# ZhiHuangHn/vtkCloudPoint

Measured on AMD Instinct MI355X. Metric: Mpoints/s DBSCAN+label @10M pts, higher is better.
Workload: dtype f64; 1 GPU; C4: 10000000-pt cloud (half uniform background, 200 Gaussian blobs), one monolithic DBImproved.dbscan, metric L1_2D, eps 0.1, minPts 10; mode=single, points_total=10000000, points_per_gpu=10000000, clusters=27380, resident_in_hbm=True

## Files before the change

vtkcloudpoint_amd/csrc/gridbuild.hip:

```cpp
#include <algorithm>
#include <mutex>
#include <unordered_map>
#include <vector>

#include "grid_common.hpp"
#include "wave.hpp"

using namespace vcpg;

namespace {

constexpr int PT = 1024;
constexpr int PCH_MIN = 8192;
constexpr int FT = 1024;
constexpr uint32_t MAXB = 8192;
constexpr uint32_t wcap(int) { return 4096u; }
constexpr uint32_t QUEUE_FROM = 32;

typedef float4 Rec;

template <int GD>
__device__ __forceinline__ Rec rec_make(const float* qf, uint32_t idx, uint32_t cell) {
  return GD == 2 ? make_float4(qf[0], qf[1], __uint_as_float(idx), __uint_as_float(cell))
                 : make_float4(qf[0], qf[1], qf[2], __uint_as_float(idx));
}
template <int GD>
__device__ __forceinline__ uint32_t rec_cell(const Rec& r, const GridP& g, uint32_t& idx) {
  if (GD == 2) {
    idx = __float_as_uint(r.z);
    return __float_as_uint(r.w);
  }
  idx = __float_as_uint(r.w);
  const float qf[3] = {r.x, r.y, r.z};
  int cc[3];
  return cell_of32<3>(qf, g, cc);
}

template <int GD>
__device__ __forceinline__ uint32_t coords_cell(const double* q, const GridP& g, float* qf) {
  int cc[3];
#pragma unroll
  for (int a = 0; a < GD; a++) qf[a] = rel32(q[a], g.mn[a], g.scale);
  return cell_of32<GD>(qf, g, cc);
}
template <int GD>
__device__ __forceinline__ uint32_t point_cell(const double* __restrict__ c, int64_t i, int stride, const GridP& g, float* qf) {
  double q[3];
  load_in<GD>(c, i, stride, q);
  return coords_cell<GD>(q, g, qf);
}

struct PartGeom {
  uint32_t csh;
  uint32_t B;
  uint32_t a;
  uint32_t NS;
  uint32_t chunk;
  uint32_t nchunk;
};

inline int env_int(const char* name, int dflt, int lo, int hi) {
  const char* e = getenv(name);
  int v = e ? atoi(e) : dflt;
  return v < lo ? lo : v > hi ? hi : v;
}

inline PartGeom part_geom(int64_t n, uint32_t ncells) {
  static const int csh_max = env_int("VCP_CPB_LOG2", 14, 10, 14);
  static const int target = env_int("VCP_PART_CHUNKS", 256, 64, 8192);
  PartGeom p;
  int csh = csh_max;
  while (csh > 10 && ((uint64_t)ncells >> csh) * 4096ull < (uint64_t)n) csh--;
  p.csh = (uint32_t)csh;
  p.B = (uint32_t)((((uint64_t)ncells + 1) + ((1ull << p.csh) - 1)) >> p.csh);
  p.a = 0;
  while (((p.B + (1u << p.a) - 1u) >> p.a) > MAXB) p.a++;
  p.NS = (p.B + (1u << p.a) - 1u) >> p.a;
  int64_t chunk = (n + target - 1) / target;
  if (chunk < PCH_MIN) chunk = PCH_MIN;
  chunk = (chunk + PT - 1) / PT * PT;
  p.chunk = (uint32_t)chunk;
  p.nchunk = (uint32_t)((n + chunk - 1) / chunk);
  return p;
}

template <int GD, bool GROUPED>
__global__ __launch_bounds__(PT) void k_part_hist(const double* __restrict__ c, int64_t n, int stride, GridP g,
                                                 const int32_t* __restrict__ group, int glo, int ghi, uint32_t csh,
                                                 uint32_t B, uint32_t chunk, uint32_t nchunk,
                                                 uint32_t* __restrict__ counts, uint32_t* __restrict__ qcount,
                                                 uint32_t* __restrict__ ctcount) {
  extern __shared__ uint32_t h[];
  if (blockIdx.x == 0 && threadIdx.x == 0) {
    *qcount = 0u;
    ctcount[0] = 0u;
  }
  for (uint32_t k = threadIdx.x; k < B; k += PT) h[k] = 0;
  __syncthreads();
  const int64_t first = (int64_t)blockIdx.x * chunk;
  const int64_t last = min(first + (int64_t)chunk, n);
#pragma unroll 4
  for (int64_t i = first + threadIdx.x; i < last; i += PT) {
    if (GROUPED) {
      const int gg = group[i];
      if (gg < glo || gg >= ghi) continue;
    }
    float qf[3];
    atomicAdd(&h[point_cell<GD>(c, i, stride, g, qf) >> csh], 1u);
  }
  __syncthreads();
  for (uint32_t k = threadIdx.x; k < B; k += PT) counts[(size_t)k * nchunk + blockIdx.x] = h[k];
}

template <int GD, bool GROUPED>
__global__ __launch_bounds__(PT) void k_part_scatter(const double* __restrict__ c, int64_t n, int stride, GridP g,
                                                    const int32_t* __restrict__ group, int glo, int ghi, uint32_t csh,
                                                    uint32_t B, uint32_t chunk, uint32_t nchunk,
                                                    const uint32_t* __restrict__ base, Rec* __restrict__ rec,
                                                    uint32_t* __restrict__ pos) {
  extern __shared__ uint32_t h[];
  for (uint32_t k = threadIdx.x; k < B; k += PT) h[k] = base[(size_t)k * nchunk + blockIdx.x];
  __syncthreads();
  const int64_t first = (int64_t)blockIdx.x * chunk;
  const int64_t last = min(first + (int64_t)chunk, n);
#pragma unroll 4
  for (int64_t i = first + threadIdx.x; i < last; i += PT) {
    if (GROUPED) {
      const int gg = group[i];
      if (gg < glo || gg >= ghi) {
        if (pos) pos[i] = NONE;
        continue;
      }
    }
    float qf[3];
    const uint32_t cell = point_cell<GD>(c, i, stride, g, qf);
    rec[atomicAdd(&h[cell >> csh], 1u)] = rec_make<GD>(qf, (uint32_t)i, cell);
  }
}

constexpr size_t PAIR_LDS = sizeof(Rec) + 8;
constexpr size_t LDS_CU = 160 * 1024;

template <int GD, bool GROUPED>
__global__ __launch_bounds__(PT) void k_part_scatter_pairs(const double* __restrict__ c, int64_t n, int stride, GridP g,
                                                          const int32_t* __restrict__ group, int glo, int ghi, uint32_t csh,
                                                          uint32_t B, uint32_t chunk, uint32_t nchunk,
                                                          const uint32_t* __restrict__ base, Rec* __restrict__ rec,
                                                          uint32_t* __restrict__ pos) {
  extern __shared__ __attribute__((aligned(16))) unsigned char lds[];
  Rec* stash = reinterpret_cast<Rec*>(lds);
  uint32_t* h = reinterpret_cast<uint32_t*>(stash + B);
  uint32_t* stash_slot = h + B;
  for (uint32_t k = threadIdx.x; k < B; k += PT) {
    h[k] = base[(size_t)k * nchunk + blockIdx.x];
    stash_slot[k] = NONE;
  }
  __syncthreads();
  const int64_t first = (int64_t)blockIdx.x * chunk;
  const int64_t last = min(first + (int64_t)chunk, n);
  const uint32_t trips = first < last ? (uint32_t)((last - first + PT - 1) / PT) : 0u;
  double nq[3] = {0.0, 0.0, 0.0};
  bool ntake = false;
  auto fetch = [&](int64_t i) {
    ntake = i < last;
    if (GROUPED && ntake) {
      const int gg = group[i];
      if (gg < glo || gg >= ghi) {
        if (pos) pos[i] = NONE;
        ntake = false;
      }
    }
    if (ntake) load_in<GD>(c, i, stride, nq);
  };
  fetch(first + threadIdx.x);
  for (uint32_t t = 0; t < trips; t++) {
    const int64_t i = first + (int64_t)t * PT + threadIdx.x;
    const bool take = ntake;
    const double q[3] = {nq[0], nq[1], nq[2]};
    fetch(i + PT);
    Rec r = make_float4(0.0f, 0.0f, 0.0f, 0.0f);
    uint32_t b = 0, slot = 0;
    if (take) {
      float qf[3];
      const uint32_t cell = coords_cell<GD>(q, g, qf);
      r = rec_make<GD>(qf, (uint32_t)i, cell);
      b = cell >> csh;
      slot = atomicAdd(&h[b], 1u);
    }
    __syncthreads();
    bool keep = false;
    if (take) {
      if (slot & 1u) {
        if (stash_slot[b] == slot - 1u) rec[slot - 1u] = stash[b];
        rec[slot] = r;
      } else if (h[b] > slot + 1u) {
        rec[slot] = r;
      } else {
        keep = true;
      }
    }
    __syncthreads();
    if (keep) {
      stash[b] = r;
      stash_slot[b] = slot;
    }
  }
  __syncthreads();
  for (uint32_t k = threadIdx.x; k < B; k += PT) {
    const uint32_t s = stash_slot[k];
    if (s != NONE && h[k] == s + 1u) rec[s] = stash[k];
  }
}

__device__ __forceinline__ uint32_t padded(uint32_t i) { return i + (i >> 5); }

template <int GD, bool GROUPED, int NT = FT>
__device__ __forceinline__ void fine_flush(uint32_t s0, uint32_t m, const float* s32, const uint32_t* sidx,
                                           const uint32_t* __restrict__ ord, const uint8_t* __restrict__ in_classed,
                                           const int32_t* __restrict__ group, float* __restrict__ sorted32,
                                           uint32_t* __restrict__ sord, uint32_t* __restrict__ sidx_out,
                                           int32_t* __restrict__ sgroup, uint8_t* __restrict__ flags,
                                           uint32_t* __restrict__ pos) {
  if (GD == 2) {
    const float2* src = reinterpret_cast<const float2*>(s32);
    float2* dst = reinterpret_cast<float2*>(sorted32) + s0;
    for (uint32_t k = threadIdx.x; k < m; k += NT) dst[k] = src[k];
  } else {
    const float4* src = reinterpret_cast<const float4*>(s32);
    float4* dst = reinterpret_cast<float4*>(sorted32) + s0;
    for (uint32_t k = threadIdx.x; k < m; k += NT) dst[k] = src[k];
  }
  for (uint32_t k = threadIdx.x; k < m; k += NT) {
    const uint32_t i = sidx[k], p = s0 + k;
    sord[p] = ord ? ord[i] : i;
    if (sidx_out) sidx_out[p] = i;
    if (GROUPED) sgroup[p] = group[i];
    if (in_classed) flags[p] = in_classed[i] ? F_CLASSED : 0;
    if (pos) pos[i] = p;
  }
}

template <int GD>
__device__ __forceinline__ void stage_put(float* s32, uint32_t* sidx, uint32_t p, const Rec& r, uint32_t idx) {
  if (GD == 2) reinterpret_cast<float2*>(s32)[p] = make_float2(r.x, r.y);
  else reinterpret_cast<float4*>(s32)[p] = make_float4(r.x, r.y, r.z, 0.0f);
  sidx[p] = idx;
}

__device__ __forceinline__ void bucket_range(const uint32_t* __restrict__ bstart, uint32_t bstride, const uint32_t* __restrict__ total,
                                             uint32_t b, uint32_t B, uint32_t& s, uint32_t& e) {
  s = bstart[(size_t)b * bstride];
  e = (b + 1 < B) ? bstart[(size_t)(b + 1) * bstride] : *total;
}

template <int GD>
__global__ __launch_bounds__(FT) void k_part_split(const Rec* __restrict__ rec, Rec* __restrict__ rec2,
                                                  const uint32_t* __restrict__ base, const uint32_t* __restrict__ total,
                                                  uint32_t nchunk, uint32_t NS, uint32_t a, uint32_t csh, uint32_t B, GridP g,
                                                  uint32_t* __restrict__ bstart) {
  __shared__ uint32_t h[32];
  const uint32_t S = blockIdx.x;
  uint32_t s, e;
  bucket_range(base, nchunk, total, S, NS, s, e);
  const uint32_t subm = (1u << a) - 1u;
  if (threadIdx.x < 32) h[threadIdx.x] = 0u;
  __syncthreads();
  for (uint32_t j = s + threadIdx.x; j < e; j += FT) {
    uint32_t i;
    atomicAdd(&h[(rec_cell<GD>(rec[j], g, i) >> csh) & subm], 1u);
  }
  __syncthreads();
  if (threadIdx.x < 32) {
    const uint32_t v = h[threadIdx.x];
    const uint32_t inc = wave_incl<WaveAdd, 32>(v, (int)threadIdx.x);
    const uint32_t first = s + inc - v;
    h[threadIdx.x] = first;
    const uint32_t bk = (S << a) + threadIdx.x;
    if (threadIdx.x <= subm && bk <= B) bstart[bk] = first;
  }
  __syncthreads();
  for (uint32_t j = s + threadIdx.x; j < e; j += FT) {
    const Rec r = rec[j];
    uint32_t i;
    rec2[atomicAdd(&h[(rec_cell<GD>(r, g, i) >> csh) & subm], 1u)] = r;
  }
}

constexpr int FS = 512;
constexpr uint32_t scap(int gd) { return gd == 2 ? 2048u : 1536u; }
constexpr uint32_t SPOP = 128;

template <int GD, bool GROUPED>
__global__ __launch_bounds__(FS) void k_part_fine_small(const Rec* __restrict__ rec, const uint32_t* __restrict__ bstart,
                                                       uint32_t bstride, const uint32_t* __restrict__ total, uint32_t B,
                                                       uint32_t csh, GridP g, const uint32_t* __restrict__ ord,
                                                       const uint8_t* __restrict__ in_classed, const int32_t* __restrict__ group,
                                                       uint4* __restrict__ ctwords, uint32_t* __restrict__ ctdense,
                                                       uint32_t* __restrict__ ctcount, uint8_t* __restrict__ bstate,
                                                       float* __restrict__ sorted32, uint32_t* __restrict__ sord,
                                                       uint32_t* __restrict__ sidx_out, int32_t* __restrict__ sgroup,
                                                       uint8_t* __restrict__ flags, uint32_t* __restrict__ pos) {
  constexpr uint32_t FPR = GD == 2 ? 2 : 4;
  constexpr uint32_t SCAP = scap(GD);
  constexpr int SRPT = SCAP / FS;
  __shared__ uint32_t ws[512 + 2];
  __shared__ uint32_t wlo[512], whi[512];
  __shared__ uint16_t wpi[512];
  __shared__ uint8_t sci[SCAP];
  __shared__ __attribute__((aligned(16))) uint16_t st32[SPOP][32];
  __shared__ __attribute__((aligned(16))) float s32[SCAP * FPR];
  __shared__ uint32_t sidx[SCAP];
  __shared__ uint32_t wsum[FS / 64];
  __shared__ uint32_t s_np, s_dbase;
  const uint32_t b = blockIdx.x;
  uint32_t s, e;
  bucket_range(bstart, bstride, total, b, B, s, e);
  const uint32_t m = e - s;
  if (b + 1 == B && threadIdx.x == 0) ctcount[1] = *total;
  if (m > SCAP) {
    if (threadIdx.x == 0) bstate[b] = 1;
    return;
  }
  const uint32_t CPB = 1u << csh, NW = CPB >> 5, c0 = b << csh;
  const int lane = threadIdx.x & 63, w = threadIdx.x >> 6;
  for (uint32_t k = threadIdx.x; k < NW + 1; k += FS) ws[k] = 0u;
  __syncthreads();
  Rec r[SRPT];
  uint32_t idx[SRPT], lw[SRPT], ci[SRPT], rnk[SRPT];
#pragma unroll
  for (int k = 0; k < SRPT; k++) {
    const uint32_t j = s + (uint32_t)k * FS + threadIdx.x;
    lw[k] = NONE;
    if (j < e) {
      r[k] = rec[j];
      const uint32_t c = rec_cell<GD>(r[k], g, idx[k]) - c0;
      lw[k] = c >> 5;
      ci[k] = c & 31u;
      rnk[k] = atomicAdd(&ws[lw[k]], 1u);
    }
  }
  __syncthreads();
  {
    const uint32_t v = threadIdx.x < NW ? ws[threadIdx.x] : 0u;
    const uint32_t inc = wave_incl<WaveAdd>(v, lane);
    if (lane == 63) wsum[w] = inc;
    __syncthreads();
    uint32_t pre = inc - v;
    for (int k = 0; k < w; k++) pre += wsum[k];
    if (threadIdx.x < NW) ws[threadIdx.x] = s + pre;
    if (threadIdx.x == 0) ws[NW] = e;
  }
  __syncthreads();
#pragma unroll
  for (int k = 0; k < SRPT; k++)
    if (lw[k] != NONE) sci[ws[lw[k]] - s + rnk[k]] = (uint8_t)ci[k];
  __syncthreads();
  bool popl = false;
  uint32_t lo = 0u, hi = 0u;
  if (threadIdx.x < NW) {
    const uint32_t a = ws[threadIdx.x] - s, k = ws[threadIdx.x + 1] - s - a;
    if (k > 64u) {
      popl = true;
    } else {
      for (uint32_t i = 0; i < k; i++) {
        const uint32_t bit = 1u << sci[a + i];
        if (lo & hi & bit) continue;
        if (lo & bit) hi ^= bit;
        lo ^= bit;
      }
      popl = (lo & hi) != 0u;
    }
  }
  {
    uint32_t tot;
    const uint32_t before = block_rank<FS>(popl, wsum, tot);
    if (threadIdx.x == 0) s_np = tot;
    if (threadIdx.x < NW) wpi[threadIdx.x] = popl ? (uint16_t)before : (uint16_t)0xFFFFu;
  }
  __syncthreads();
  const uint32_t np = s_np;
  if (np > SPOP) {
    if (threadIdx.x == 0) bstate[b] = 1;
    return;
  }
  if (threadIdx.x == 0) {
    bstate[b] = 0;
    s_dbase = np ? atomicAdd(&ctcount[0], np) : 0u;
  }
  for (uint32_t k = threadIdx.x; k < np * 16u; k += FS) reinterpret_cast<uint32_t*>(&st32[0][0])[k] = 0u;
  if (threadIdx.x < NW && !popl) {
    wlo[threadIdx.x] = lo;
    whi[threadIdx.x] = hi;
  }
  __syncthreads();
#pragma unroll
  for (int k = 0; k < SRPT; k++)
    if (lw[k] != NONE && wpi[lw[k]] != 0xFFFFu) {
      uint16_t* c = &st32[wpi[lw[k]]][ci[k]];
      atomicAdd(reinterpret_cast<uint32_t*>(reinterpret_cast<uintptr_t>(c) & ~(uintptr_t)3), ((uintptr_t)c & 2) ? 0x10000u : 1u);
    }
  __syncthreads();
  {
    const uint32_t hw = threadIdx.x >> 5, li = threadIdx.x & 31u;
    for (uint32_t wd = hw; wd < NW; wd += FS / 32) {
      const uint32_t pi = wpi[wd];
      if (pi == 0xFFFFu) continue;
      const uint32_t c = st32[pi][li];
      uint32_t inc = c;
#pragma unroll
      for (int d = 1; d < 32; d <<= 1) {
        const uint32_t t = __shfl_up(inc, d, 32);
        if ((int)li >= d) inc += t;
      }
      const uint32_t first = ws[wd] + inc - c;
      st32[pi][li] = (uint16_t)(first - s);
      ctdense[(size_t)(s_dbase + pi) * 32u + li] = first;
      const uint32_t cs = min(c, 3u);
      const unsigned long long blo = __ballot(cs & 1u), bhi = __ballot(cs >> 1);
      const int sh = (threadIdx.x & 32) ? 32 : 0;
      if (li == 0) {
        wlo[wd] = (uint32_t)(blo >> sh);
        whi[wd] = (uint32_t)(bhi >> sh);
      }
    }
  }
  __syncthreads();
#pragma unroll
  for (int k = 0; k < SRPT; k++) {
    if (lw[k] == NONE) continue;
    const uint32_t pi = wpi[lw[k]];
    uint32_t p;
    if (pi != 0xFFFFu) {
      uint16_t* c = &st32[pi][ci[k]];
      const bool up = ((uintptr_t)c & 2) != 0;
      const uint32_t old = atomicAdd(reinterpret_cast<uint32_t*>(reinterpret_cast<uintptr_t>(c) & ~(uintptr_t)3), up ? 0x10000u : 1u);
      p = up ? old >> 16 : old & 0xFFFFu;
    } else {
      const uint32_t l = wlo[lw[k]], h = whi[lw[k]], below = (1u << ci[k]) - 1u;
      const uint32_t a = ws[lw[k]] - s;
      p = a + (uint32_t)__popc(l & below) + 2u * (uint32_t)__popc(h & below);
      if ((h >> ci[k]) & 1u)
        for (uint32_t i = 0; i < rnk[k]; i++) p += sci[a + i] == (uint8_t)ci[k] ? 1u : 0u;
    }
    stage_put<GD>(s32, sidx, p, r[k], idx[k]);
  }
  if (threadIdx.x < NW) {
    const size_t W = (size_t)(c0 >> 5) + threadIdx.x;
    const uint32_t pi = wpi[threadIdx.x];
    if (W < vcp_ct_words(g.ncells))
      ctwords[W] = make_uint4(wlo[threadIdx.x], whi[threadIdx.x], ws[threadIdx.x], pi != 0xFFFFu ? s_dbase + pi : NONE);
  }
  __syncthreads();
  fine_flush<GD, GROUPED, FS>(s, m, s32, sidx, ord, in_classed, group, sorted32, sord, sidx_out, sgroup, flags, pos);
}

constexpr uint32_t mcap(int gd) { return gd == 2 ? 8192u : 4096u; }
constexpr uint32_t mstg(int gd) { return gd == 2 ? 2048u : 1024u; }
constexpr size_t mid_lds(int gd, uint32_t cpb) { return (size_t)cpb * 2 + (size_t)mstg(gd) * ((gd == 2 ? 8 : 16) + 4); }

__device__ __forceinline__ uint32_t mid_slot(uint32_t c, uint32_t half) {
  return ((c >> 3) & 1u) * half + ((c >> 4) << 3) + (c & 7u);
}

template <int GD, bool GROUPED>
__global__ __launch_bounds__(FT, 8) void k_part_fine_mid(const Rec* __restrict__ rec, const uint32_t* __restrict__ bstart,
                                                     uint32_t bstride, const uint32_t* __restrict__ total, uint32_t B,
                                                     uint32_t csh, GridP g, const uint32_t* __restrict__ ord,
                                                     const uint8_t* __restrict__ in_classed, const int32_t* __restrict__ group,
                                                     uint4* __restrict__ ctwords, uint32_t* __restrict__ ctdense,
                                                     uint32_t* __restrict__ ctcount, uint8_t* __restrict__ bstate,
                                                     float* __restrict__ sorted32, uint32_t* __restrict__ sord,
                                                     uint32_t* __restrict__ sidx_out, int32_t* __restrict__ sgroup,
                                                     uint8_t* __restrict__ flags, uint32_t* __restrict__ pos) {
  extern __shared__ __attribute__((aligned(16))) unsigned char lds[];
  __shared__ uint32_t wsum[FT / 64];
  __shared__ uint32_t w_lo[512], w_hi[512], w_slot[512];
  __shared__ uint32_t s_dbase;
  constexpr uint32_t WCAP = mcap(GD), STG = mstg(GD);
  constexpr uint32_t FPR = GD == 2 ? 2 : 4;
  constexpr int MRPT = WCAP / FT;
  static_assert(WCAP % FT == 0 && WCAP % STG == 0 && WCAP <= 0xFFFFu, "k_part_fine_mid: window shape");
  const uint32_t b = blockIdx.x;
  if (bstate[b] != 1) return;
  uint32_t s, e;
  bucket_range(bstart, bstride, total, b, B, s, e);
  const uint32_t m = e - s;
  if (m > WCAP || m == 0u) return;
  const uint32_t CPB = 1u << csh, HALF = CPB >> 1, c0 = b << csh;
  uint32_t* cnt = reinterpret_cast<uint32_t*>(lds);
  float* s32 = reinterpret_cast<float*>(lds + (size_t)CPB * 2);
  uint32_t* sidx = reinterpret_cast<uint32_t*>(s32 + (size_t)STG * FPR);
  Rec r[MRPT];
  uint32_t idx[MRPT], cl[MRPT];
  __shared__ uint32_t park[MRPT / 2][FT];
#pragma unroll
  for (int k = 0; k < MRPT; k++) {
    const uint32_t j = s + (uint32_t)k * FT + threadIdx.x;
    r[k] = rec[min(j, e - 1u)];
  }
#pragma unroll
  for (int k = 0; k < MRPT; k++) {
    const uint32_t c = rec_cell<GD>(r[k], g, idx[k]) - c0;
    cl[k] = s + (uint32_t)k * FT + threadIdx.x < e ? c : NONE;
    if (k >= MRPT / 2) park[k - MRPT / 2][threadIdx.x] = idx[k];
  }
  uint4* cnt4 = reinterpret_cast<uint4*>(lds);
  for (uint32_t k = threadIdx.x; k < CPB / 8; k += FT) cnt4[k] = make_uint4(0u, 0u, 0u, 0u);
  __syncthreads();
#pragma unroll
  for (int k = 0; k < MRPT; k++)
    if (cl[k] != NONE) atomicAdd(&cnt[mid_slot(cl[k], HALF) >> 1], (cl[k] & 1u) ? 0x10000u : 1u);
  __syncthreads();
  const uint32_t NA = CPB >> 4, NW = CPB >> 5;
  const bool act = threadIdx.x < NA;
  uint32_t loc = 0;
  if (act) {
    const uint4 a = cnt4[threadIdx.x], c = cnt4[NA + threadIdx.x];
    loc = a.x + a.y + a.z + a.w + c.x + c.y + c.z + c.w;
    loc = (loc & 0xFFFFu) + (loc >> 16);
  }
  uint32_t pre = block_excl(loc, wsum);
  {
    const uint32_t wstart = s + pre, bit0 = (threadIdx.x & 1u) << 4;
    uint32_t plo = 0u, phi = 0u;
#pragma unroll
    for (int h = 0; h < 2; h++) {
      uint4 a = make_uint4(0u, 0u, 0u, 0u);
      if (act) a = cnt4[h * NA + threadIdx.x];
      uint32_t v[4] = {a.x, a.y, a.z, a.w};
#pragma unroll
      for (int k = 0; k < 4; k++) {
        const uint32_t n0 = v[k] & 0xFFFFu, n1 = v[k] >> 16;
        v[k] = pre | ((pre + n0) << 16);
        pre += n0 + n1;
        const uint32_t q0 = min(n0, 3u), q1 = min(n1, 3u);
        plo |= ((q0 & 1u) | ((q1 & 1u) << 1)) << (bit0 + 8 * h + 2 * k);
        phi |= ((q0 >> 1) | ((q1 >> 1) << 1)) << (bit0 + 8 * h + 2 * k);
      }
      if (act) cnt4[h * NA + threadIdx.x] = make_uint4(v[0], v[1], v[2], v[3]);
    }
    plo |= (uint32_t)__shfl_xor((int)plo, 1, 64);
    phi |= (uint32_t)__shfl_xor((int)phi, 1, 64);
    if (act && (threadIdx.x & 1u) == 0u) {
      w_lo[threadIdx.x >> 1] = plo;
      w_hi[threadIdx.x >> 1] = phi;
      w_slot[threadIdx.x >> 1] = wstart;
    }
  }
  __syncthreads();
  {
    const bool popl = threadIdx.x < NW && (w_lo[threadIdx.x] & w_hi[threadIdx.x]) != 0u;
    uint32_t tot;
    const uint32_t before = block_rank<FT>(popl, wsum, tot);
    if (threadIdx.x == 0) {
      s_dbase = tot ? atomicAdd(&ctcount[0], tot) : 0u;
      bstate[b] = 2;
    }
    __syncthreads();
    if (threadIdx.x < NW) {
      const uint32_t slot = popl ? s_dbase + before : NONE;
      const uint32_t wpos = w_slot[threadIdx.x];
      w_slot[threadIdx.x] = slot;
      const size_t W = (size_t)(c0 >> 5) + threadIdx.x;
      if (W < vcp_ct_words(g.ncells))
        ctwords[W] = make_uint4(w_lo[threadIdx.x], w_hi[threadIdx.x], wpos, slot);
    }
    __syncthreads();
    const uint16_t* cnt16 = reinterpret_cast<const uint16_t*>(lds);
    const uint32_t hw = threadIdx.x >> 5, li = threadIdx.x & 31u;
    for (uint32_t j = hw; j < NW; j += FT / 32) {
      const uint32_t slot = w_slot[j];
      if (slot != NONE) ctdense[(size_t)slot * 32u + li] = s + cnt16[mid_slot(32u * j + li, HALF)];
    }
  }
  __syncthreads();
#pragma unroll
  for (int k = 0; k < MRPT; k++) {
    if (cl[k] != NONE) {
      const bool up = (cl[k] & 1u) != 0u;
      const uint32_t old = atomicAdd(&cnt[mid_slot(cl[k], HALF) >> 1], up ? 0x10000u : 1u);
      cl[k] = up ? old >> 16 : old & 0xFFFFu;
    }
  }
  for (uint32_t w0 = 0; w0 < m; w0 += STG) {
#pragma unroll
    for (int k = 0; k < MRPT; k++) {
      const uint32_t q = cl[k] - w0;
      if (q < STG) stage_put<GD>(s32, sidx, q, r[k], k >= MRPT / 2 ? park[k - MRPT / 2][threadIdx.x] : idx[k]);
    }
    __syncthreads();
    fine_flush<GD, GROUPED>(s + w0, min(STG, m - w0), s32, sidx, ord, in_classed, group, sorted32, sord, sidx_out, sgroup,
                            flags, pos);
    __syncthreads();
  }
}

template <int GD, bool GROUPED>
__global__ __launch_bounds__(FT) void k_part_fine(const Rec* __restrict__ rec, uint32_t* __restrict__ rk,
                                                 const uint32_t* __restrict__ bstart, uint32_t bstride,
                                                 const uint32_t* __restrict__ total, uint32_t B, uint32_t csh, GridP g,
                                                 const uint32_t* __restrict__ ord, const uint8_t* __restrict__ in_classed,
                                                 const int32_t* __restrict__ group, uint4* __restrict__ ctwords,
                                                 uint32_t* __restrict__ ctdense, uint32_t* __restrict__ ctcount,
                                                 float* __restrict__ sorted32, uint32_t* __restrict__ sord,
                                                 uint32_t* __restrict__ sidx_out, int32_t* __restrict__ sgroup,
                                                 uint8_t* __restrict__ flags, uint32_t* __restrict__ pos,
                                                 uint2* __restrict__ queue, uint32_t* __restrict__ qcount,
                                                 const uint8_t* __restrict__ bstate) {
  extern __shared__ __attribute__((aligned(16))) unsigned char lds[];
  __shared__ uint32_t wsum[FT / 64];
  __shared__ uint32_t w_lo[512], w_hi[512], w_slot[512];
  __shared__ uint32_t s_dbase;
  const uint32_t b = blockIdx.x;
  if (bstate[b] != 1) return;
  constexpr uint32_t WCAP = wcap(GD);
  constexpr uint32_t FPR = GD == 2 ? 2 : 4;
  const uint32_t CPB = 1u << csh;
  uint32_t* cnt = reinterpret_cast<uint32_t*>(lds);
  float* s32 = reinterpret_cast<float*>(lds + (((size_t)padded(CPB) + 4) & ~3ull) * 4);
  uint32_t* sidx = reinterpret_cast<uint32_t*>(s32 + (size_t)WCAP * FPR);
  const uint32_t c0 = b << csh;
  uint32_t s, e;
  bucket_range(bstart, bstride, total, b, B, s, e);
  const uint32_t m = e - s;
  const bool big = m > WCAP;
  for (uint32_t k = threadIdx.x; k < padded(CPB); k += FT) cnt[k] = 0;
  __syncthreads();
  for (uint32_t j = s + threadIdx.x; j < e; j += FT) {
    uint32_t i;
    uint32_t* slot = &cnt[padded(rec_cell<GD>(rec[j], g, i) - c0)];
    if (big) rk[j] = atomicAdd(slot, 1u);
    else atomicAdd(slot, 1u);
  }
  __syncthreads();
  const uint32_t PER = CPB / FT;
  const uint32_t first = threadIdx.x * PER;
  uint32_t loc = 0;
  for (uint32_t k = 0; k < PER; k++) loc += cnt[padded(first + k)];
  uint32_t pre = block_excl(loc, wsum, s);
  const uint32_t NW = CPB >> 5;
  uint32_t plo = 0u, phi = 0u;
  const uint32_t wstart = pre;
  {
    const uint32_t bit0 = first & 31u;
    for (uint32_t k = 0; k < PER; k++) {
      const uint32_t v = cnt[padded(first + k)];
      cnt[padded(first + k)] = pre;
      pre += v;
      const uint32_t c = min(v, 3u);
      plo |= (c & 1u) << (bit0 + k);
      phi |= (c >> 1) << (bit0 + k);
    }
    for (uint32_t d = 1; d < 32u / PER; d <<= 1) {
      plo |= (uint32_t)__shfl_xor((int)plo, (int)d, 64);
      phi |= (uint32_t)__shfl_xor((int)phi, (int)d, 64);
    }
    if ((first & 31u) == 0u) {
      w_lo[first >> 5] = plo;
      w_hi[first >> 5] = phi;
      w_slot[first >> 5] = wstart;
    }
  }
  __syncthreads();
  {
    const bool popl = threadIdx.x < NW && (w_lo[threadIdx.x] & w_hi[threadIdx.x]) != 0u;
    uint32_t tot;
    const uint32_t before = block_rank<FT>(popl, wsum, tot);
    if (threadIdx.x == 0) s_dbase = tot ? atomicAdd(&ctcount[0], tot) : 0u;
    __syncthreads();
    if (threadIdx.x < NW) {
      const uint32_t slot = popl ? s_dbase + before : NONE;
      const uint32_t wpos = w_slot[threadIdx.x];
      w_slot[threadIdx.x] = slot;
      const size_t W = (size_t)(c0 >> 5) + threadIdx.x;
      if (W < vcp_ct_words(g.ncells))
        ctwords[W] = make_uint4(w_lo[threadIdx.x], w_hi[threadIdx.x], wpos, slot);
    }
    __syncthreads();
    const uint32_t hw = threadIdx.x >> 5, li = threadIdx.x & 31u;
    for (uint32_t j = hw; j < NW; j += FT / 32) {
      const uint32_t slot = w_slot[j];
      if (slot != NONE) ctdense[(size_t)slot * 32u + li] = cnt[padded(32u * j + li)];
    }
  }
  __syncthreads();
  if (!big) {
    for (uint32_t j = s + threadIdx.x; j < e; j += FT) {
      const Rec r = rec[j];
      uint32_t i;
      const uint32_t p = atomicAdd(&cnt[padded(rec_cell<GD>(r, g, i) - c0)], 1u) - s;
      stage_put<GD>(s32, sidx, p, r, i);
    }
    __syncthreads();
    fine_flush<GD, GROUPED>(s, m, s32, sidx, ord, in_classed, group, sorted32, sord, sidx_out, sgroup, flags, pos);
    return;
  }
  if (m > QUEUE_FROM * WCAP) {
    __shared__ uint32_t q0;
    const uint32_t nwin = (m + WCAP - 1) / WCAP;
    if (threadIdx.x == 0) q0 = atomicAdd(qcount, nwin);
    __syncthreads();
    for (uint32_t k = threadIdx.x; k < nwin; k += FT) queue[q0 + k] = make_uint2(b, k * WCAP);
    return;
  }
  for (uint32_t w0 = 0; w0 < m; w0 += WCAP) {
    for (uint32_t j = s + threadIdx.x; j < e; j += FT) {
      const Rec r = rec[j];
      uint32_t i;
      const uint32_t p = cnt[padded(rec_cell<GD>(r, g, i) - c0)] + rk[j] - s - w0;
      if (p < WCAP) stage_put<GD>(s32, sidx, p, r, i);
    }
    __syncthreads();
    fine_flush<GD, GROUPED>(s + w0, min(WCAP, m - w0), s32, sidx, ord, in_classed, group, sorted32, sord, sidx_out, sgroup,
                            flags, pos);
    __syncthreads();
  }
}

template <int GD, bool GROUPED>
__global__ __launch_bounds__(FT) void k_part_fine_windows(const Rec* __restrict__ rec, const uint32_t* __restrict__ rk,
                                                         const uint32_t* __restrict__ bstart, uint32_t bstride,
                                                         const uint32_t* __restrict__ total, uint32_t B, GridP g,
                                                         const uint32_t* __restrict__ ord, const uint8_t* __restrict__ in_classed,
                                                         const int32_t* __restrict__ group, CellTab ct,
                                                         float* __restrict__ sorted32,
                                                         uint32_t* __restrict__ sord, uint32_t* __restrict__ sidx_out,
                                                         int32_t* __restrict__ sgroup, uint8_t* __restrict__ flags,
                                                         uint32_t* __restrict__ pos, const uint2* __restrict__ queue,
                                                         const uint32_t* __restrict__ qcount) {
  extern __shared__ __attribute__((aligned(16))) unsigned char lds[];
  constexpr uint32_t WCAP = wcap(GD);
  constexpr uint32_t FPR = GD == 2 ? 2 : 4;
  float* s32 = reinterpret_cast<float*>(lds);
  uint32_t* sidx = reinterpret_cast<uint32_t*>(s32 + (size_t)WCAP * FPR);
  const uint32_t nq = *qcount;
  for (uint32_t qi = blockIdx.x; qi < nq; qi += gridDim.x) {
    const uint2 q = queue[qi];
    const uint32_t b = q.x, w0 = q.y;
    uint32_t s, e;
    bucket_range(bstart, bstride, total, b, B, s, e);
    const uint32_t m = e - s;
    for (uint32_t j = s + threadIdx.x; j < e; j += FT) {
      const Rec r = rec[j];
      uint32_t i;
      const uint32_t p = ct_start(ct, rec_cell<GD>(r, g, i)) + rk[j] - s - w0;
      if (p < WCAP) stage_put<GD>(s32, sidx, p, r, i);
    }
    __syncthreads();
    fine_flush<GD, GROUPED>(s + w0, min(WCAP, m - w0), s32, sidx, ord, in_classed, group, sorted32, sord, sidx_out, sgroup,
                            flags, pos);
    __syncthreads();
  }
}

constexpr int OT = 1024, OPT = 10;
constexpr int OWT = 512;

template <int OWSH>
__global__ __launch_bounds__(OT, 8) void k_out_scatter(const uint32_t* __restrict__ sord, const uint32_t* __restrict__ labk,
                                                   int64_t n, uint32_t OB, uint32_t* __restrict__ gcur,
                                                   uint2* __restrict__ rec) {
  extern __shared__ uint32_t h[];
  for (uint32_t k = threadIdx.x; k < OB; k += OT) h[k] = 0;
  __syncthreads();
  const int64_t first = (int64_t)blockIdx.x * (OT * OPT);
  static_assert(OPT % 2 == 0 && OT * OPT <= 65536, "k_out_scatter: packed ranks");
  uint32_t o[OPT], w[OPT], r[OPT / 2];
  const uint32_t cnt = (uint32_t)min((int64_t)(OT * OPT), n - first);
  const uint32_t* __restrict__ so = sord + first;
  const uint32_t* __restrict__ la = labk + first;
#pragma unroll
  for (int k = 0; k < OPT; k++) {
    const uint32_t q = min((uint32_t)k * OT + threadIdx.x, cnt - 1u);
    o[k] = so[q];
    w[k] = la[q];
  }
#pragma unroll
  for (int k = 0; k < OPT / 2; k++) r[k] = 0u;
#pragma unroll
  for (int k = 0; k < OPT; k++) {
    if ((uint32_t)k * OT + threadIdx.x < cnt) r[k >> 1] |= atomicAdd(&h[o[k] >> OWSH], 1u) << (16 * (k & 1));
    else o[k] = NONE;
  }
  __syncthreads();
  for (uint32_t k = threadIdx.x; k < OB; k += OT) {
    const uint32_t c = h[k];
    if (c) h[k] = atomicAdd(&gcur[k], c);
  }
  __syncthreads();
#pragma unroll
  for (int k = 0; k < OPT; k++) {
    if (o[k] == NONE) continue;
    const uint32_t bk = o[k] >> OWSH;
    rec[((size_t)bk << OWSH) + h[bk] + ((r[k >> 1] >> (16 * (k & 1))) & 0xFFFFu)] = make_uint2(o[k], w[k]);
  }
}

template <int OWSH>
__global__ __launch_bounds__(OWT) void k_out_write(const uint2* __restrict__ rec, int64_t n, bool have_in_classed,
                                                  int32_t cf_in, int32_t* __restrict__ labels,
                                                  uint8_t* __restrict__ is_core, uint8_t* __restrict__ is_classed,
                                                  unsigned long long* __restrict__ counters, uint32_t* __restrict__ gcur) {
  extern __shared__ __attribute__((aligned(16))) uint32_t sw[];
  if (threadIdx.x == 0) gcur[blockIdx.x] = 0u;
  const int64_t lo = (int64_t)blockIdx.x << OWSH;
  const uint32_t cnt = (uint32_t)min((int64_t)1 << OWSH, n - lo);
  unsigned unclassed = 0;
  for (uint32_t j = threadIdx.x; j < cnt; j += OWT) {
    const uint2 v = rec[lo + j];
    sw[v.x - (uint32_t)lo] = v.y;
    if (!(v.y & 2u)) unclassed++;
  }
  __syncthreads();
  auto lab_of = [&](uint32_t w) { return (w >> 2) ? cf_in + (int32_t)(w >> 2) : 0; };
  auto core_of = [](uint32_t w) { return (uint32_t)((w & 3u) == 1u); };
  auto cls_of = [](uint32_t w) { return (uint32_t)((w & 2u) != 0u || (w >> 2) != 0u); };
  const bool vec = (((uintptr_t)labels & 15u) | ((uintptr_t)is_core & 3u) | ((uintptr_t)is_classed & 3u)) == 0;
  const uint32_t c4 = vec ? cnt >> 2 : 0u;
  for (uint32_t j = threadIdx.x; j < c4; j += OWT) {
    const uint4 w = reinterpret_cast<const uint4*>(sw)[j];
    const int4 l = make_int4(lab_of(w.x), lab_of(w.y), lab_of(w.z), lab_of(w.w));
    if (have_in_classed) {
      if (l.x) labels[lo + 4 * j] = l.x;
      if (l.y) labels[lo + 4 * j + 1] = l.y;
      if (l.z) labels[lo + 4 * j + 2] = l.z;
      if (l.w) labels[lo + 4 * j + 3] = l.w;
    } else {
      reinterpret_cast<int4*>(labels + lo)[j] = l;
    }
    if (is_core)
      reinterpret_cast<uint32_t*>(is_core + lo)[j] = core_of(w.x) | core_of(w.y) << 8 | core_of(w.z) << 16 | core_of(w.w) << 24;
    if (is_classed)
      reinterpret_cast<uint32_t*>(is_classed + lo)[j] = cls_of(w.x) | cls_of(w.y) << 8 | cls_of(w.z) << 16 | cls_of(w.w) << 24;
  }
  for (uint32_t j = (c4 << 2) + threadIdx.x; j < cnt; j += OWT) {
    const uint32_t w = sw[j];
    const int32_t l = lab_of(w);
    if (!have_in_classed || l) labels[lo + j] = l;
    if (is_core) is_core[lo + j] = (uint8_t)core_of(w);
    if (is_classed) is_classed[lo + j] = (uint8_t)cls_of(w);
  }
  if (have_in_classed) {
    __shared__ unsigned wc[OWT / 64];
#pragma unroll
    for (int d = 32; d > 0; d >>= 1) unclassed += __shfl_down(unclassed, d, 64);
    if ((threadIdx.x & 63) == 0) wc[threadIdx.x >> 6] = unclassed;
    __syncthreads();
    if (threadIdx.x == 0) {
      unsigned t = 0;
      for (int k = 0; k < OWT / 64; k++) t += wc[k];
      if (t) atomicAdd(&counters[CNT_UNCLASSED + (blockIdx.x & (CNT_SPREAD - 1))], (unsigned long long)t);
    }
  }
}

int allow_lds(vcp_ctx* ctx, const void* kernel, size_t bytes) {
  static std::mutex mu;
  static std::unordered_map<uint64_t, size_t> allowed;
  std::lock_guard<std::mutex> lk(mu);
  const uint64_t key = (uint64_t)reinterpret_cast<uintptr_t>(kernel) * 64u + (uint64_t)(ctx->device & 63);
  size_t& have = allowed.emplace(key, (size_t)64 * 1024).first->second;
  if (bytes > have) {
    VCP_HIP(ctx, hipFuncSetAttribute(kernel, hipFuncAttributeMaxDynamicSharedMemorySize, (int)bytes));
    have = bytes;
  }
  return VCP_OK;
}
template <class K>
int allow_lds(vcp_ctx* ctx, K kernel, size_t bytes) {
  return allow_lds(ctx, reinterpret_cast<const void*>(kernel), bytes);
}

template <int GD, bool GROUPED>
int build(vcp_ctx* ctx, const GridBuildArgs& a) {
  hipStream_t st = ctx->stream;
  const PartGeom pg = part_geom(a.n, a.g.ncells);
  const size_t nc = (size_t)pg.NS * pg.nchunk;
  VCP_TRY(vcp_ensure(ctx, ctx->b_hist, (nc + 8) * 4));
  VCP_TRY(vcp_ensure(ctx, ctx->b_rec, (size_t)a.n * sizeof(Rec)));
  uint32_t* counts = ctx->b_hist.as<uint32_t>();
  uint32_t* total = counts + nc;
  Rec* rec = ctx->b_rec.as<Rec>();
  const size_t lds_h = (size_t)pg.NS * 4;
  const uint32_t CPB = 1u << pg.csh;
  const size_t lds_f = ((((size_t)CPB + CPB / 32) + 4) & ~3ull) * 4 + (size_t)wcap(GD) * ((GD == 2 ? 8 : 16) + 4);
  VCP_TRY(allow_lds(ctx, k_part_fine<GD, GROUPED>, lds_f));
  VCP_TRY(vcp_ensure(ctx, ctx->b_fineq, ((size_t)a.n / wcap(GD) + pg.B + 8) * sizeof(uint2) + 64));
  uint32_t* qcount = ctx->b_fineq.as<uint32_t>();
  uint2* queue = reinterpret_cast<uint2*>(ctx->b_fineq.as<char>() + 64);
  vcp_phase(ctx, "part_hist");
  const uint32_t csh_a = pg.csh + pg.a;
  VCP_LAUNCH(ctx, (k_part_hist<GD, GROUPED>), dim3(pg.nchunk), dim3(PT), lds_h, st, a.d_coords, a.n, a.stride, a.g,
                  a.d_group, a.glo, a.ghi, csh_a, pg.NS, pg.chunk, pg.nchunk, counts, qcount, a.ctcount);
  VCP_TRY(vcp_exclusive_scan_u32(ctx, counts, counts, (int64_t)nc, total));
  vcp_phase(ctx, "part_scatter");
  static const bool pairs_on = env_int("VCP_PART_PAIRS", 1, 0, 1) != 0;
  const size_t lds_p = (size_t)pg.NS * PAIR_LDS;
  if (vcp_trace_on())
    vcp_trace_line("gridbuild scatter pairs_on=%d NS=%u lds_p=%zu stash=%d", (int)pairs_on, (unsigned)pg.NS, lds_p,
                   (int)(pairs_on && lds_p <= LDS_CU));
  if (pairs_on && lds_p <= LDS_CU) {
    if (reinterpret_cast<uintptr_t>(rec) & 31u)
      return vcp_fail(ctx, VCP_ERR_HIP, "the record array is not 32-byte aligned");
    VCP_TRY(allow_lds(ctx, k_part_scatter_pairs<GD, GROUPED>, lds_p));
    VCP_LAUNCH(ctx, (k_part_scatter_pairs<GD, GROUPED>), dim3(pg.nchunk), dim3(PT), lds_p, st, a.d_coords, a.n, a.stride,
                    a.g, a.d_group, a.glo, a.ghi, csh_a, pg.NS, pg.chunk, pg.nchunk, counts, rec, a.pos);
  } else {
    VCP_LAUNCH(ctx, (k_part_scatter<GD, GROUPED>), dim3(pg.nchunk), dim3(PT), lds_h, st, a.d_coords, a.n, a.stride, a.g,
                    a.d_group, a.glo, a.ghi, csh_a, pg.NS, pg.chunk, pg.nchunk, counts, rec, a.pos);
  }
  const uint32_t* bstart = counts;
  uint32_t bstride = pg.nchunk;
  if (pg.a > 0) {
    vcp_phase(ctx, "part_split");
    VCP_TRY(vcp_ensure(ctx, ctx->b_rec2, (size_t)a.n * sizeof(Rec)));
    VCP_TRY(vcp_ensure(ctx, ctx->b_bstart, ((size_t)pg.B + 2) * 4));
    VCP_LAUNCH(ctx, k_part_split<GD>, dim3(pg.NS), dim3(FT), 0, st, rec, ctx->b_rec2.as<Rec>(), counts, total, pg.nchunk,
                    pg.NS, pg.a, pg.csh, pg.B, a.g, ctx->b_bstart.as<uint32_t>());
    rec = ctx->b_rec2.as<Rec>();
    bstart = ctx->b_bstart.as<uint32_t>();
    bstride = 1;
  }
  vcp_phase(ctx, "part_fine");
  VCP_TRY(vcp_ensure(ctx, ctx->b_rank, (size_t)a.n * 4));
  VCP_TRY(vcp_ensure(ctx, ctx->b_bstate, (size_t)pg.B + 16));
  uint8_t* bstate = ctx->b_bstate.as<uint8_t>();
  VCP_LAUNCH(ctx, (k_part_fine_small<GD, GROUPED>), dim3(pg.B), dim3(FS), 0, st, rec, bstart, bstride, total, pg.B, pg.csh,
                  a.g, a.d_ord, a.d_in_classed, a.d_group, a.ctwords, a.ctdense, a.ctcount, bstate, a.sorted32, a.sord,
                  a.sidx, a.sgroup, a.flags, a.pos);
  static const bool mid_env = env_int("VCP_FINE_MID", 1, 0, 1) != 0;
  const bool mid_on = mid_env && GD == 2;
  const size_t lds_m = mid_lds(GD, CPB);
  if (vcp_trace_on()) vcp_trace_line("gridfine mid_on=%d lds_m=%zu", (int)mid_on, lds_m);
  if constexpr (GD == 2) if (mid_on) {
    VCP_TRY(allow_lds(ctx, k_part_fine_mid<GD, GROUPED>, lds_m));
    VCP_LAUNCH(ctx, (k_part_fine_mid<GD, GROUPED>), dim3(pg.B), dim3(FT), lds_m, st, rec, bstart, bstride, total, pg.B,
                    pg.csh, a.g, a.d_ord, a.d_in_classed, a.d_group, a.ctwords, a.ctdense, a.ctcount, bstate, a.sorted32,
                    a.sord, a.sidx, a.sgroup, a.flags, a.pos);
  }
  VCP_LAUNCH(ctx, (k_part_fine<GD, GROUPED>), dim3(pg.B), dim3(FT), lds_f, st, rec, ctx->b_rank.as<uint32_t>(), bstart,
                  bstride, total, pg.B, pg.csh, a.g, a.d_ord, a.d_in_classed, a.d_group, a.ctwords, a.ctdense, a.ctcount,
                  a.sorted32, a.sord, a.sidx, a.sgroup, a.flags, a.pos, queue, qcount, bstate);
  {
    const size_t lds_w = (size_t)wcap(GD) * ((GD == 2 ? 8 : 16) + 4);
    VCP_TRY(allow_lds(ctx, k_part_fine_windows<GD, GROUPED>, lds_w));
    const unsigned gw = (unsigned)std::min<size_t>(768, (size_t)a.n / wcap(GD) + 1);
    const CellTab ct{a.ctwords, a.ctdense, a.ctcount + 1};
    VCP_LAUNCH(ctx, (k_part_fine_windows<GD, GROUPED>), dim3(gw), dim3(FT), lds_w, st, rec, ctx->b_rank.as<uint32_t>(),
                    bstart, bstride, total, pg.B, a.g, a.d_ord, a.d_in_classed, a.d_group, ct, a.sorted32,
                    a.sord, a.sidx, a.sgroup, a.flags, a.pos, queue, qcount);
  }
  if (vcp_trace_on()) {
    std::vector<uint8_t> hs(pg.B);
    VCP_HIP(ctx, hipMemcpyAsync(hs.data(), bstate, pg.B, hipMemcpyDeviceToHost, st));
    VCP_HIP(ctx, hipStreamSynchronize(st));
    unsigned cnt[3] = {0u, 0u, 0u};
    for (uint8_t v : hs) cnt[v < 3 ? v : 1]++;
    vcp_trace_line("gridfine small=%u mid=%u big=%u", cnt[0], cnt[2], cnt[1]);
  }
  return VCP_OK;
}

}

int vcp_grid_build_partition(vcp_ctx* ctx, const GridBuildArgs& a) {
  const bool grouped = a.d_group != nullptr;
  if (a.gd == 3) {
    if (grouped) return vcp_fail(ctx, VCP_ERR_ARG, "grouped calls are 2-D");
    return build<3, false>(ctx, a);
  }
  return grouped ? build<2, true>(ctx, a) : build<2, false>(ctx, a);
}

template <int OWSH>
static int output_partition(vcp_ctx* ctx, const GridOutputArgs& a) {
  hipStream_t st = ctx->stream;
  const uint32_t OB = (uint32_t)((a.n + (1 << OWSH) - 1) >> OWSH);
  const void* before = ctx->b_outcur.p;
  const size_t before_cap = ctx->b_outcur.cap;
  VCP_TRY(vcp_ensure(ctx, ctx->b_outcur, ((size_t)OB + 8) * 4));
  if (ctx->b_outcur.p != before || ctx->b_outcur.cap != before_cap)
    VCP_HIP(ctx, hipMemsetAsync(ctx->b_outcur.p, 0, ctx->b_outcur.cap, st));
  VCP_TRY(vcp_ensure(ctx, ctx->b_rec, (size_t)OB << (OWSH + 3)));
  uint32_t* gcur = ctx->b_outcur.as<uint32_t>();
  uint2* rec = ctx->b_rec.as<uint2>();
  VCP_TRY(allow_lds(ctx, k_out_write<OWSH>, (size_t)4 << OWSH));
  vcp_phase(ctx, "out_scatter");
  VCP_LAUNCH(ctx, k_out_scatter<OWSH>, dim3(vcp_blocks(a.n, OT * OPT)), dim3(OT), (size_t)OB * 4, st, a.sord, a.labk, a.n,
                  OB, gcur, rec);
  vcp_phase(ctx, "out_write");
  VCP_LAUNCH(ctx, k_out_write<OWSH>, dim3(OB), dim3(OWT), (size_t)4 << OWSH, st, rec, a.n, a.have_in_classed, a.cf_in,
                  a.labels, a.is_core, a.is_classed, a.counters, gcur);
  return VCP_OK;
}

int vcp_grid_output_partition(vcp_ctx* ctx, const GridOutputArgs& a) {
  if (a.n > ((int64_t)1 << 27)) return vcp_fail(ctx, VCP_ERR_TOO_LARGE, "more than 2^27 points: use the gather output");
  if (a.n >= ((int64_t)1 << 23)) return output_partition<15>(ctx, a);
  if (a.n >= ((int64_t)1 << 22)) return output_partition<14>(ctx, a);
  return output_partition<13>(ctx, a);
}
```

Baseline: 7766 Mpoints/s.

## Stream oversized buckets through the mid fine-partition kernel instead of big path

Extends k_part_fine_mid so that buckets larger than its register window (up to 65535 points) are handled by streaming the records twice: a first pass builds the per-cell counts in LDS, and after the cell table is written a second pass reloads the records and scatters each one directly to its final sorted position with atomics. These buckets previously fell through to the heavier k_part_fine and window path with its global queue. The cell-table construction is factored out into a helper, and streamed buckets are marked with a new bstate value. The cost is that every record is read and its cell recomputed twice, and the direct global scatter is uncoalesced and its order within a cell is nondeterministic.

```diff
diff --git a/vtkcloudpoint_amd/csrc/gridbuild.hip b/vtkcloudpoint_amd/csrc/gridbuild.hip
--- a/vtkcloudpoint_amd/csrc/gridbuild.hip
+++ b/vtkcloudpoint_amd/csrc/gridbuild.hip
@@ -463,9 +463,94 @@
 }
 
 template <int GD, bool GROUPED>
+__device__ __forceinline__ void fine_put(uint32_t p, const Rec& r, uint32_t i, const uint32_t* __restrict__ ord,
+                                         const uint8_t* __restrict__ in_classed, const int32_t* __restrict__ group,
+                                         float* __restrict__ sorted32, uint32_t* __restrict__ sord,
+                                         uint32_t* __restrict__ sidx_out, int32_t* __restrict__ sgroup,
+                                         uint8_t* __restrict__ flags, uint32_t* __restrict__ pos) {
+  if (GD == 2) reinterpret_cast<float2*>(sorted32)[p] = make_float2(r.x, r.y);
+  else reinterpret_cast<float4*>(sorted32)[p] = make_float4(r.x, r.y, r.z, 0.0f);
+  sord[p] = ord ? ord[i] : i;
+  if (sidx_out) sidx_out[p] = i;
+  if (GROUPED) sgroup[p] = group[i];
+  if (in_classed) flags[p] = in_classed[i] ? F_CLASSED : 0;
+  if (pos) pos[i] = p;
+}
+
+__device__ __forceinline__ void mid_table(unsigned char* lds, uint32_t* wsum, uint32_t* w_lo, uint32_t* w_hi, uint32_t* w_slot,
+                                          uint32_t* s_dbase, uint32_t CPB, uint32_t s, uint32_t c0, uint32_t b, const GridP& g,
+                                          uint4* __restrict__ ctwords, uint32_t* __restrict__ ctdense,
+                                          uint32_t* __restrict__ ctcount, uint8_t* __restrict__ bstate, uint8_t mark) {
+  uint4* cnt4 = reinterpret_cast<uint4*>(lds);
+  const uint32_t HALF = CPB >> 1;
+  const uint32_t NA = CPB >> 4, NW = CPB >> 5;
+  const bool act = threadIdx.x < NA;
+  uint32_t loc = 0;
+  if (act) {
+    const uint4 a = cnt4[threadIdx.x], c = cnt4[NA + threadIdx.x];
+    loc = a.x + a.y + a.z + a.w + c.x + c.y + c.z + c.w;
+    loc = (loc & 0xFFFFu) + (loc >> 16);
+  }
+  uint32_t pre = block_excl(loc, wsum);
+  {
+    const uint32_t wstart = s + pre, bit0 = (threadIdx.x & 1u) << 4;
+    uint32_t plo = 0u, phi = 0u;
+#pragma unroll
+    for (int h = 0; h < 2; h++) {
+      uint4 a = make_uint4(0u, 0u, 0u, 0u);
+      if (act) a = cnt4[h * NA + threadIdx.x];
+      uint32_t v[4] = {a.x, a.y, a.z, a.w};
+#pragma unroll
+      for (int k = 0; k < 4; k++) {
+        const uint32_t n0 = v[k] & 0xFFFFu, n1 = v[k] >> 16;
+        v[k] = pre | ((pre + n0) << 16);
+        pre += n0 + n1;
+        const uint32_t q0 = min(n0, 3u), q1 = min(n1, 3u);
+        plo |= ((q0 & 1u) | ((q1 & 1u) << 1)) << (bit0 + 8 * h + 2 * k);
+        phi |= ((q0 >> 1) | ((q1 >> 1) << 1)) << (bit0 + 8 * h + 2 * k);
+      }
+      if (act) cnt4[h * NA + threadIdx.x] = make_uint4(v[0], v[1], v[2], v[3]);
+    }
+    plo |= (uint32_t)__shfl_xor((int)plo, 1, 64);
+    phi |= (uint32_t)__shfl_xor((int)phi, 1, 64);
+    if (act && (threadIdx.x & 1u) == 0u) {
+      w_lo[threadIdx.x >> 1] = plo;
+      w_hi[threadIdx.x >> 1] = phi;
+      w_slot[threadIdx.x >> 1] = wstart;
+    }
+  }
+  __syncthreads();
+  {
+    const bool popl = threadIdx.x < NW && (w_lo[threadIdx.x] & w_hi[threadIdx.x]) != 0u;
+    uint32_t tot;
+    const uint32_t before = block_rank<FT>(popl, wsum, tot);
+    if (threadIdx.x == 0) {
+      *s_dbase = tot ? atomicAdd(&ctcount[0], tot) : 0u;
+      bstate[b] = mark;
+    }
+    __syncthreads();
+    if (threadIdx.x < NW) {
+      const uint32_t slot = popl ? *s_dbase + before : NONE;
+      const uint32_t wpos = w_slot[threadIdx.x];
+      w_slot[threadIdx.x] = slot;
+      const size_t W = (size_t)(c0 >> 5) + threadIdx.x;
+      if (W < vcp_ct_words(g.ncells))
+        ctwords[W] = make_uint4(w_lo[threadIdx.x], w_hi[threadIdx.x], wpos, slot);
+    }
+    __syncthreads();
+    const uint16_t* cnt16 = reinterpret_cast<const uint16_t*>(lds);
+    const uint32_t hw = threadIdx.x >> 5, li = threadIdx.x & 31u;
+    for (uint32_t j = hw; j < NW; j += FT / 32) {
+      const uint32_t slot = w_slot[j];
+      if (slot != NONE) ctdense[(size_t)slot * 32u + li] = s + cnt16[mid_slot(32u * j + li, HALF)];
+    }
+  }
+}
+
+template <int GD, bool GROUPED>
 __global__ __launch_bounds__(FT, 8) void k_part_fine_mid(const Rec* __restrict__ rec, const uint32_t* __restrict__ bstart,
                                                      uint32_t bstride, const uint32_t* __restrict__ total, uint32_t B,
-                                                     uint32_t csh, GridP g, const uint32_t* __restrict__ ord,
+                                                     uint32_t csh, uint32_t mmax, GridP g, const uint32_t* __restrict__ ord,
                                                      const uint8_t* __restrict__ in_classed, const int32_t* __restrict__ group,
                                                      uint4* __restrict__ ctwords, uint32_t* __restrict__ ctdense,
                                                      uint32_t* __restrict__ ctcount, uint8_t* __restrict__ bstate,
@@ -485,95 +570,70 @@
   uint32_t s, e;
   bucket_range(bstart, bstride, total, b, B, s, e);
   const uint32_t m = e - s;
-  if (m > WCAP || m == 0u) return;
+  if (m > mmax || m == 0u) return;
   const uint32_t CPB = 1u << csh, HALF = CPB >> 1, c0 = b << csh;
   uint32_t* cnt = reinterpret_cast<uint32_t*>(lds);
+  uint4* cnt4 = reinterpret_cast<uint4*>(lds);
+  const bool stream = m > WCAP;
   float* s32 = reinterpret_cast<float*>(lds + (size_t)CPB * 2);
   uint32_t* sidx = reinterpret_cast<uint32_t*>(s32 + (size_t)STG * FPR);
   Rec r[MRPT];
   uint32_t idx[MRPT], cl[MRPT];
   __shared__ uint32_t park[MRPT / 2][FT];
-#pragma unroll
-  for (int k = 0; k < MRPT; k++) {
-    const uint32_t j = s + (uint32_t)k * FT + threadIdx.x;
-    r[k] = rec[min(j, e - 1u)];
-  }
-#pragma unroll
-  for (int k = 0; k < MRPT; k++) {
-    const uint32_t c = rec_cell<GD>(r[k], g, idx[k]) - c0;
-    cl[k] = s + (uint32_t)k * FT + threadIdx.x < e ? c : NONE;
-    if (k >= MRPT / 2) park[k - MRPT / 2][threadIdx.x] = idx[k];
-  }
-  uint4* cnt4 = reinterpret_cast<uint4*>(lds);
-  for (uint32_t k = threadIdx.x; k < CPB / 8; k += FT) cnt4[k] = make_uint4(0u, 0u, 0u, 0u);
-  __syncthreads();
-#pragma unroll
-  for (int k = 0; k < MRPT; k++)
-    if (cl[k] != NONE) atomicAdd(&cnt[mid_slot(cl[k], HALF) >> 1], (cl[k] & 1u) ? 0x10000u : 1u);
-  __syncthreads();
-  const uint32_t NA = CPB >> 4, NW = CPB >> 5;
-  const bool act = threadIdx.x < NA;
-  uint32_t loc = 0;
-  if (act) {
-    const uint4 a = cnt4[threadIdx.x], c = cnt4[NA + threadIdx.x];
-    loc = a.x + a.y + a.z + a.w + c.x + c.y + c.z + c.w;
-    loc = (loc & 0xFFFFu) + (loc >> 16);
-  }
-  uint32_t pre = block_excl(loc, wsum);
-  {
-    const uint32_t wstart = s + pre, bit0 = (threadIdx.x & 1u) << 4;
-    uint32_t plo = 0u, phi = 0u;
-#pragma unroll
-    for (int h = 0; h < 2; h++) {
-      uint4 a = make_uint4(0u, 0u, 0u, 0u);
-      if (act) a = cnt4[h * NA + threadIdx.x];
-      uint32_t v[4] = {a.x, a.y, a.z, a.w};
-#pragma unroll
-      for (int k = 0; k < 4; k++) {
-        const uint32_t n0 = v[k] & 0xFFFFu, n1 = v[k] >> 16;
-        v[k] = pre | ((pre + n0) << 16);
-        pre += n0 + n1;
-        const uint32_t q0 = min(n0, 3u), q1 = min(n1, 3u);
-        plo |= ((q0 & 1u) | ((q1 & 1u) << 1)) << (bit0 + 8 * h + 2 * k);
-        phi |= ((q0 >> 1) | ((q1 >> 1) << 1)) << (bit0 + 8 * h + 2 * k);
+  if (stream) {
+    for (uint32_t k = threadIdx.x; k < CPB / 8; k += FT) cnt4[k] = make_uint4(0u, 0u, 0u, 0u);
+    __syncthreads();
+    for (uint32_t j0 = s; j0 < e; j0 += WCAP) {
+      Rec q[MRPT];
+#pragma unroll
+      for (int k = 0; k < MRPT; k++) q[k] = rec[min(j0 + (uint32_t)k * FT + threadIdx.x, e - 1u)];
+#pragma unroll
+      for (int k = 0; k < MRPT; k++) {
+        uint32_t i;
+        const uint32_t c = rec_cell<GD>(q[k], g, i) - c0;
+        if (j0 + (uint32_t)k * FT + threadIdx.x < e) atomicAdd(&cnt[mid_slot(c, HALF) >> 1], (c & 1u) ? 0x10000u : 1u);
       }
-      if (act) cnt4[h * NA + threadIdx.x] = make_uint4(v[0], v[1], v[2], v[3]);
-    }
-    plo |= (uint32_t)__shfl_xor((int)plo, 1, 64);
-    phi |= (uint32_t)__shfl_xor((int)phi, 1, 64);
-    if (act && (threadIdx.x & 1u) == 0u) {
-      w_lo[threadIdx.x >> 1] = plo;
-      w_hi[threadIdx.x >> 1] = phi;
-      w_slot[threadIdx.x >> 1] = wstart;
-    }
-  }
-  __syncthreads();
-  {
-    const bool popl = threadIdx.x < NW && (w_lo[threadIdx.x] & w_hi[threadIdx.x]) != 0u;
-    uint32_t tot;
-    const uint32_t before = block_rank<FT>(popl, wsum, tot);
-    if (threadIdx.x == 0) {
-      s_dbase = tot ? atomicAdd(&ctcount[0], tot) : 0u;
-      bstate[b] = 2;
-    }
-    __syncthreads();
-    if (threadIdx.x < NW) {
-      const uint32_t slot = popl ? s_dbase + before : NONE;
-      const uint32_t wpos = w_slot[threadIdx.x];
-      w_slot[threadIdx.x] = slot;
-      const size_t W = (size_t)(c0 >> 5) + threadIdx.x;
-      if (W < vcp_ct_words(g.ncells))
-        ctwords[W] = make_uint4(w_lo[threadIdx.x], w_hi[threadIdx.x], wpos, slot);
-    }
-    __syncthreads();
-    const uint16_t* cnt16 = reinterpret_cast<const uint16_t*>(lds);
-    const uint32_t hw = threadIdx.x >> 5, li = threadIdx.x & 31u;
-    for (uint32_t j = hw; j < NW; j += FT / 32) {
-      const uint32_t slot = w_slot[j];
-      if (slot != NONE) ctdense[(size_t)slot * 32u + li] = s + cnt16[mid_slot(32u * j + li, HALF)];
-    }
-  }
-  __syncthreads();
+    }
+  } else {
+#pragma unroll
+    for (int k = 0; k < MRPT; k++) {
+      const uint32_t j = s + (uint32_t)k * FT + threadIdx.x;
+      r[k] = rec[min(j, e - 1u)];
+    }
+#pragma unroll
+    for (int k = 0; k < MRPT; k++) {
+      const uint32_t c = rec_cell<GD>(r[k], g, idx[k]) - c0;
+      cl[k] = s + (uint32_t)k * FT + threadIdx.x < e ? c : NONE;
+      if (k >= MRPT / 2) park[k - MRPT / 2][threadIdx.x] = idx[k];
+    }
+    for (uint32_t k = threadIdx.x; k < CPB / 8; k += FT) cnt4[k] = make_uint4(0u, 0u, 0u, 0u);
+    __syncthreads();
+#pragma unroll
+    for (int k = 0; k < MRPT; k++)
+      if (cl[k] != NONE) atomicAdd(&cnt[mid_slot(cl[k], HALF) >> 1], (cl[k] & 1u) ? 0x10000u : 1u);
+  }
+  __syncthreads();
+  mid_table(lds, wsum, w_lo, w_hi, w_slot, &s_dbase, CPB, s, c0, b, g, ctwords, ctdense, ctcount, bstate, stream ? 3 : 2);
+  __syncthreads();
+  if (stream) {
+    for (uint32_t j0 = s; j0 < e; j0 += WCAP) {
+      Rec q[MRPT];
+#pragma unroll
+      for (int k = 0; k < MRPT; k++) q[k] = rec[min(j0 + (uint32_t)k * FT + threadIdx.x, e - 1u)];
+#pragma unroll
+      for (int k = 0; k < MRPT; k++) {
+        uint32_t i;
+        const uint32_t c = rec_cell<GD>(q[k], g, i) - c0;
+        if (j0 + (uint32_t)k * FT + threadIdx.x < e) {
+          const bool up = (c & 1u) != 0u;
+          const uint32_t old = atomicAdd(&cnt[mid_slot(c, HALF) >> 1], up ? 0x10000u : 1u);
+          fine_put<GD, GROUPED>(s + (up ? old >> 16 : old & 0xFFFFu), q[k], i, ord, in_classed, group, sorted32, sord,
+                                sidx_out, sgroup, flags, pos);
+        }
+      }
+    }
+    return;
+  }
 #pragma unroll
   for (int k = 0; k < MRPT; k++) {
     if (cl[k] != NONE) {
@@ -932,11 +992,14 @@
   const bool mid_on = mid_env && GD == 2;
   const size_t lds_m = mid_lds(GD, CPB);
   if (vcp_trace_on()) vcp_trace_line("gridfine mid_on=%d lds_m=%zu", (int)mid_on, lds_m);
+  static const bool stream_env = env_int("VCP_FINE_STREAM", 1, 0, 1) != 0;
+  const bool stream_on = mid_on && stream_env;
+  if (vcp_trace_on()) vcp_trace_line("gridfine stream_on=%d", (int)stream_on);
   if constexpr (GD == 2) if (mid_on) {
     VCP_TRY(allow_lds(ctx, k_part_fine_mid<GD, GROUPED>, lds_m));
     VCP_LAUNCH(ctx, (k_part_fine_mid<GD, GROUPED>), dim3(pg.B), dim3(FT), lds_m, st, rec, bstart, bstride, total, pg.B,
-                    pg.csh, a.g, a.d_ord, a.d_in_classed, a.d_group, a.ctwords, a.ctdense, a.ctcount, bstate, a.sorted32,
-                    a.sord, a.sidx, a.sgroup, a.flags, a.pos);
+                    pg.csh, stream_on ? 0xFFFFu : mcap(GD), a.g, a.d_ord, a.d_in_classed, a.d_group, a.ctwords, a.ctdense,
+                    a.ctcount, bstate, a.sorted32, a.sord, a.sidx, a.sgroup, a.flags, a.pos);
   }
   VCP_LAUNCH(ctx, (k_part_fine<GD, GROUPED>), dim3(pg.B), dim3(FT), lds_f, st, rec, ctx->b_rank.as<uint32_t>(), bstart,
                   bstride, total, pg.B, pg.csh, a.g, a.d_ord, a.d_in_classed, a.d_group, a.ctwords, a.ctdense, a.ctcount,
@@ -954,9 +1017,13 @@
     std::vector<uint8_t> hs(pg.B);
     VCP_HIP(ctx, hipMemcpyAsync(hs.data(), bstate, pg.B, hipMemcpyDeviceToHost, st));
     VCP_HIP(ctx, hipStreamSynchronize(st));
-    unsigned cnt[3] = {0u, 0u, 0u};
-    for (uint8_t v : hs) cnt[v < 3 ? v : 1]++;
+    unsigned cnt[3] = {0u, 0u, 0u}, streamed = 0u;
+    for (uint8_t v : hs) {
+      cnt[v < 3 ? v : 1]++;
+      streamed += v == 3 ? 1u : 0u;
+    }
     vcp_trace_line("gridfine small=%u mid=%u big=%u", cnt[0], cnt[2], cnt[1]);
+    vcp_trace_line("gridfine streamed=%u", streamed);
   }
   return VCP_OK;
 }
```

New measurement: 7893 Mpoints/s (median of 6 runs). +1.6%, better.
